# xtcyclist/hash_join_codes_KNL

Measured on AMD Instinct MI355X. Metric: probe Gtuples/s + % HBM roofline, PHJ |R|=64M join |S|=1G, 1/2/4/8 GPU, higher is better.
Workload: dtype u32

## Files before the change

hash_join_codes_knl_amd/csrc/hj_internal.hpp:

```cpp
#pragma once
#include <hip/hip_runtime.h>
#include <stdint.h>
#include <type_traits>
#include "../../include/hjgpu.h"

typedef unsigned long long u64;

constexpr uint32_t HJ_LINE_TUPLES = 16;
constexpr uint32_t HJ_STREAM_UNIT = 256;
constexpr uint32_t HJ_MAX_HEAVY = 128;
struct ScatterConfig { int block, vpt; bool carry; };
struct HjTuning;
ScatterConfig hj_scatter_config(const HjTuning &t, int pass, uint32_t F, bool out_packed);
int hj_scatter_tile(const HjTuning &t, int pass, uint32_t F, bool out_packed);
constexpr int HJ_JOIN_SLICE    = 1 << 16;
constexpr int HJ_JOIN_FILL_GROUPS = 64;
inline size_t hj_join_items_capacity(size_t partitions, size_t outer_rows)
{
    return (partitions + outer_rows / HJ_JOIN_SLICE + 1) * HJ_JOIN_FILL_GROUPS;
}

struct JoinConfig {
    int block, log2slots, batch;
    int slots() const { return 1 << log2slots; }
// ... 8 lines not shown
    bool npj_refhash = false;
    bool no_broadcast = false;
    bool force_chained = false;
    bool scatter_prof = false;
    bool unique = false;
    bool piece_interleave = true;
    bool merged_plan = true;
    int placement = 12;
    int placement_ms = 500;
    bool placement_log = false;
    bool exact_probe_counts = false;
    int probe_slack = 12;
    bool solo = false;
    bool audit = false;
    int hist_min_lds = 0;
    int reserve_cus = 0;
    long long host_batch = -1;
    long long group_from = 300000000, group_inner = 64000000;
    bool group_always = false;
    bool group_device = true;
    int group_slack = 50;
    long long batch_tuples = 0;
    JoinConfig join = {512, 13, 2};
    int scatter_cfg[2][3] = {{0, 0, -1}, {0, 0, -1}};
};
void hj_tuning_from_env(HjTuning *t);
bool hj_tuning_set(HjTuning *t, const char *name, const char *value);
inline const JoinConfig &hj_join_config_of(const HjTuning &t, bool big_tables) { return big_tables ? hj_join_config_big() : t.join; }

struct HjPerDeviceOnce { unsigned char done[64]; };
int hj_allow_dynamic_lds(const void *kernel, int bytes, HjPerDeviceOnce *once);

constexpr uint32_t HJ_MAX_RANGE_ENTRIES = 1u << 24;
constexpr uint32_t HJ_MAX_CHUNKS = 256;
constexpr uint32_t HJ_TICKET_K4 = 0;
constexpr uint32_t HJ_TICKET_K6 = 2 * HJ_MAX_CHUNKS;
constexpr uint32_t HJ_TICKET_MULTI_FILL = 2 * HJ_MAX_CHUNKS + 8;
constexpr uint32_t HJ_TICKET_JOIN = 2 * HJ_MAX_CHUNKS + 10;
constexpr uint32_t HJ_TICKET_JOIN2 = 2 * HJ_MAX_CHUNKS + 12;
constexpr uint32_t HJ_TICKET_JOIN3 = 2 * HJ_MAX_CHUNKS + 14;
constexpr uint32_t HJ_TICKET_WORDS = 2 * HJ_MAX_CHUNKS + 16;
struct Pass1Geom {
    u64 n, part;
#if defined(__HIPCC__)
    __host__ __device__
#endif
    u64 beg(uint32_t c) const { return c >= chunks ? n : part * c; }
    uint32_t chunks;
    uint32_t align;
    uint32_t ranges_per_chunk;
    uint32_t tile;
};
#if defined(__HIPCC__)
__host__ __device__
#endif
inline u64 hj_tiles_of(u64 b, u64 e, uint32_t align, uint32_t tile)
{
    if (e <= b) return 0;
    const u64 gb = (align + b) & ~3ull, ge = align + e;
    return (ge - gb + tile - 1) / tile;
}

struct ScatterArgs {
    const uint32_t *kin, *vin;
// ... 132 lines not shown
int hj_launch_group_result(const hjgpu_result *state, const uint32_t *skew, hjgpu_result *d_result, hipStream_t stream);
int hj_launch_range_base(const uint32_t *range_counts, const u64 *off1, u64 *range_base,
                         uint32_t chunks, uint32_t ranges_per_chunk, uint32_t F1, hipStream_t stream,
                         uint32_t own_first = 0, uint32_t own_count = 0, uint32_t group_bins = 0);
__host__ __device__ inline u64 hj_group_shift(u64 dense_start, uint32_t g)
{
    return ((dense_start + 31) & ~(u64)31) - dense_start + (u64)32 * g;
}
int hj_launch_plan(const PlanArgs &a, hipStream_t stream);
int hj_launch_claimed_pieces(const u64 *off2, const u64 *end2, const u64 *cur2, uint32_t P, u64 *pieces_beg, u64 *pieces_end, hipStream_t stream);
int hj_launch_claimed_desc(const u64 *claim_cursors, u64 cap1, uint32_t F1, uint32_t F2, uint32_t tile2, uint4 *tdesc, uint32_t tdesc_cap,
                           u64 *total, uint32_t *overflow, hipStream_t stream);
struct BatchPlanArgs {
    const uint32_t *range_counts;
    u64 *range_base;
    u64 *boff;
    u64 *tp2b;
    uint4 *tdesc;
    uint32_t tdesc_cap;
    uint32_t ranges, ranges_per_batch, F1, F2, tile2;
};
int hj_launch_batch_plan(const BatchPlanArgs &a, uint32_t batches, hipStream_t stream);
int hj_launch_scatter(const ScatterArgs &a, const HjTuning &t, int cus, hipStream_t stream);
int hj_launch_join(const JoinArgs &a, const HjTuning &t, int cus, hipStream_t stream);
int hj_launch_exscan(const u64 *in, u64 *out, uint32_t n, hipStream_t stream);
int hj_launch_offsets_to_counts(const u64 *off, u64 *counts, uint32_t P, hipStream_t stream);

template <class F>
inline void hj_with_bool(bool b, F &&f)
{
    if (b) f(std::true_type{});
    else f(std::false_type{});
}

int hj_launch_npj_build(const uint32_t *keys, const uint32_t *vals, size_t n, u64 *table,
                        size_t buckets, uint32_t factor, uint32_t *zero_key_flag,
                        int cus, hipStream_t stream, bool line_hash = false);
struct NpjProbeArgs {
    const uint32_t *keys, *vals;
    size_t n;
    const u64 *table;
    size_t buckets;
    uint32_t factor;
    uint32_t line_hash;
    uint32_t unique;
    uint32_t mode;
    hjgpu_result *result;
// ... 104 lines not shown
```

hash_join_codes_knl_amd/csrc/hjgpu_api.hip:

```cpp
#include "hjgpu_ctx.hpp"
#include "hj_device.hpp"

using namespace hjapi;



namespace hjapi {


int fail(hjgpu_ctx *ctx, int status, const char *what, hipError_t e)
{
    if (ctx) {
        if (e != hipSuccess)
            snprintf(ctx->err, sizeof(ctx->err), "%s: %s", what, hipGetErrorString(e));
        else
            snprintf(ctx->err, sizeof(ctx->err), "%s", what);
    }
    return status;
}

static int release(hjgpu_ctx *ctx, void *p)
{
    if (!p) return HJGPU_OK;
    HIPCHK(ctx, hipFree(p));
// ... 160 lines not shown
        m.cur1[r] = take((size_t)C * F1);
        m.tp1[r] = take(C + 1);
        m.seg1[r] = take(C + 1);
        m.tp2[r] = take((size_t)C * F1 + 1);
        m.seg2[r] = take((size_t)F1 + 1);
        m.more[r] = C > 8 ? take(P) : nullptr;
    }
    m.claim_total = take(1);
    m.pieces = take((size_t)4 * P);
    m.slice_prefix = take((size_t)P + 1);
    m.slices = take(P);
    m.item_part = reinterpret_cast<uint32_t *>(take(((size_t)P + items_extra + 2) / 2 + 1));
    for (int r = 0; r < 2; ++r) {
        m.range_counts[r] = reinterpret_cast<uint32_t *>(take((ranges * F1 + 1) / 2));
        m.range_base[r] = take(ranges * F1);
    }
    m.tdesc_cap = tiles2;
    for (int r = 0; r < 2; ++r) m.tdesc[r] = reinterpret_cast<uint4 *>(take(tiles2 * 4));
    m.boff = take(batches * ((size_t)F1 + 1));
    m.tp2b = take(batches * ((size_t)F1 + 1));
    m.tdescb = reinterpret_cast<uint4 *>(take(batches * tdesc_b_cap * 4));
    m.btickets = reinterpret_cast<uint32_t *>(take(batches + 1));
    m.btickets_bytes = (batches + 1) * sizeof(u64);
    m.total_bytes = at * sizeof(u64);
    return m;
}

void choose_fanout(const HjTuning &tune, size_t inner, const hjgpu_phj_params *prm, uint32_t *F1, uint32_t *F2, bool *big_tables)
{
    uint32_t f1 = prm ? prm->fanout1 : 0, f2 = prm ? prm->fanout2 : 0;
    *big_tables = false;
    if (f1 == 0) {
        double target = tune.join.cap() * 0.85;
        double parts = ceil((double)inner / target);
        if (parts > HJGPU_MAX_PARTS) {
            *big_tables = true;
            target = hj_join_config_big().cap() * 0.85;
            parts = ceil((double)inner / target);
        }
        if (parts < 64) parts = 64;
        if (parts > HJGPU_MAX_PARTS) parts = HJGPU_MAX_PARTS;
        if (parts <= 640) { f1 = (uint32_t)parts; f2 = 1; }
        else {
            f1 = 2;
            while ((double)f1 * f1 * 2.0 < parts) f1 <<= 1;
            if (f1 > 256) f1 = 256;
// ... 644 lines not shown
        }
        ja.slice_prefix = m.slice_prefix; ja.slices = m.slices; ja.item_part = m.item_part;
        ja.P = pl.P; ja.chunks = road.pad2 ? 1u : pl.C;
        ja.f1 = pl.f1; ja.F1 = pl.F1; ja.f2 = pl.f2; ja.F2 = pl.F2;
        if (o.pre) { ja.f1 = pl.pre_f1; ja.F1 = pl.pre_F1tot; ja.p1_base = pl.pre_base; }
        ja.tf0 = pl.tf0; ja.tf1 = pl.tf1;
        ja.s_align = 0;
        ja.packed = 1;
        ja.big_tables = pl.big_tables ? 1u : 0u;
        ja.unique = pl.first_match ? 1u : 0u;
        ja.mode = pl.mode;
        ja.result = &st->result;
        ja.work_counter = reinterpret_cast<u64 *>(m.tickets + HJ_TICKET_JOIN);
        ja.work_counter2 = reinterpret_cast<u64 *>(m.tickets + HJ_TICKET_JOIN2);
        ja.work_counter3 = reinterpret_cast<u64 *>(m.tickets + HJ_TICKET_JOIN3);
        ja.multi_fill = m.tickets + HJ_TICKET_MULTI_FILL;
        ja.resume = o.grp ? 1u : 0u;
        join_output(ctx, ja, o.out, bs, bl, st);
        if (marks) {
            ja.build_bits = reinterpret_cast<uint32_t *>(ctx->build_bits.p);
            HIPCHK(ctx, hj_zero_async(ja.build_bits, build_bits_bytes(pl, nn[0]), stream));
            if ((!nn[1] || build_rows) && bs && !o.grp) HIPCHK(ctx, hj_fill_async(ctx->final_offsets.p, 0xFFFFFFFFu, (size_t)workers * sizeof(u64), stream));
        }
        if (nn[1]) CHK(hj_launch_join(ja, ctx->tune, ctx->cus, stream));
        if (build_rows) CHK(hj_launch_build_rows(ja, ctx->tune, ctx->cus, stream));
        else if (marks) CHK(hj_launch_build_unmatched(ja, ctx->tune, ctx->cus, stream));
        if (audit) CHK(hj_audit_copy(reinterpret_cast<const u64 *>(&st->result), audit + 4 * 6, 4, stream));
        return HJGPU_OK;
    }
};

}

int phj_enqueue(hjgpu_ctx *ctx, const PhjPlan &pl, const Rel &R, const Rel &S, hipStream_t stream, const EnqueueOpts &o)
{
    CHK(refuse_capture(ctx, stream));
    if (o.grp && (o.pre || o.stages != PHJ_WHOLE || o.inner_ready)) return fail(ctx, HJGPU_EINVAL, "internal: a device-planned group is a whole join on resident columns");
    if ((o.pre != nullptr) != (pl.pre != 0)) return fail(ctx, HJGPU_EINVAL, "internal: plan and relations disagree about pre-partitioning");
    PhjRun run(ctx, pl, R, S, o, stream);
    const uint32_t workers = (uint32_t)hj_join_workers(ctx->tune, ctx->cus, pl.big_tables);
    u64 bs = 0, bl = 0;
    CHK(setup_output(ctx, o.out, workers, &bs, &bl, pl.mode));

    CHK(run.setup());
    record(ctx, EV_BEGIN, stream);
    CHK(run.begin());
    CHK(run.road.merged ? run.partition_merged() : run.partition_in_turn());
    if (hj_mode_marks_build(pl.mode) && (o.pre || o.stages != PHJ_WHOLE)) return fail(ctx, HJGPU_EINVAL, "internal: a join that marks its build rows is a whole join");
    if (run.road.joins) CHK(run.join(bs, bl, workers));
    record(ctx, EV_JOIN, stream);
    if (bs && run.road.joins && !o.grp) CHK(close_gaps(ctx, o.out, workers, bs, run.st, stream, pl.mode));
    record(ctx, EV_GAPS, stream);
    ctx->stats.fanout1 = pl.F1; ctx->stats.fanout2 = pl.F2; ctx->stats.buckets = 0; ctx->stats.batches = run.batches_used;
    ctx->last_algo = 1;
    return HJGPU_OK;
}

static int finish_from(hjgpu_ctx *ctx, const DevState &h, hjgpu_result *result, const hjgpu_output *out)
{
    if (result) *result = h.result;
    if (h.zero_key) return fail(ctx, HJGPU_EZEROKEY, "NPJ: a build key is 0, the empty-bucket sentinel");
    if (h.overflow) return fail(ctx, HJGPU_EOVERFLOW, "materialised output exceeded its capacity");
    if (out && out->d_keys && h.dense != h.result.count && (h.result.count != 0 || h.dense != 0))
        return fail(ctx, HJGPU_EHIP, "internal: dense length != match count after close_gaps");
    return HJGPU_OK;
}

static int read_state(hjgpu_ctx *ctx, DevState &h, hipStream_t stream)
{
    HIPCHK(ctx, hipMemcpyAsync(&h, ctx->state.p, sizeof(DevState), hipMemcpyDeviceToHost, stream));
    HIPCHK(ctx, hipStreamSynchronize(stream));
    return HJGPU_OK;
}

int finish_blocking(hjgpu_ctx *ctx, hjgpu_result *result, const hjgpu_output *out, hipStream_t stream)
{
    DevState h;
    CHK(read_state(ctx, h, stream));
    return finish_from(ctx, h, result, out);
}

static bool claimed_probe_allowed(const hjgpu_ctx *ctx)
{
// ... 302 lines not shown
    const uint32_t groups = grouped_groups(ctx, inner, outer, nullptr);
    if (groups > 1 && outer) {
        ReserveClock clock(ctx);
        size_t cap_r, cap_s, plan_inner;
        grouped_caps(ctx, groups, inner, outer, &cap_r, &cap_s, &plan_inner);
        CHK(grouped_twins(ctx, group_layout(groups), inner, outer));
        CHK(phj_prepare(ctx, cap_r, cap_s, &prm, 8, &pl, {.plan_inner = plan_inner}));
    } else {
        CHK(phj_prepare(ctx, inner, outer, &prm, 8, &pl));
        if (claimed_probe_allowed(ctx)) CHK(phj_prepare(ctx, inner, outer, &prm, 1, &pl, {.claim_s = true}));
    }
    size_t buckets; uint32_t factor;
    CHK(npj_prepare(ctx, inner, nullptr, &buckets, &factor));
    return HJGPU_OK;
}

static size_t lds_lookup_rows(const HjTuning &tune);
int hjgpu_get_counter(hjgpu_ctx *ctx, const char *name, uint64_t *value)
{
    if (!ctx || !name || !value) return HJGPU_EINVAL;
    if (strcmp(name, "probe_fallbacks") == 0) { *value = ctx->probe_fallbacks; return HJGPU_OK; }
    if (strcmp(name, "probe_exact") == 0) { *value = (ctx->tune.exact_probe_counts || ctx->probe_exact) ? 1u : 0u; return HJGPU_OK; }
    if (strcmp(name, "lookup_lds_rows") == 0) { *value = lds_lookup_rows(ctx->tune); return HJGPU_OK; }
    return fail(ctx, HJGPU_EINVAL, "unknown counter (probe_fallbacks, probe_exact, lookup_lds_rows)");
}

static void fill_reserve(const hjgpu_ctx *ctx, hjgpu_stats *s)
{
    s->ms_reserve = ctx->ms_reserve;
    s->placement_tried = ctx->placement_tried; s->placement_timeboxed = ctx->placement_timeboxed;
    s->placement_fill_ms = ctx->placement_fill_ms; s->placement_search_ms = ctx->placement_search_ms; s->placement_bytes = (uint64_t)ctx->placement_bytes;
}

int hjgpu_get_stats(hjgpu_ctx *ctx, hjgpu_stats *s)
{
    if (!ctx || !s) return HJGPU_EINVAL;
    if (ctx->stats_override) {
        *s = ctx->stats;
        fill_reserve(ctx, s);
        return HJGPU_OK;
    }
    if (ctx->grp_ev_groups) {
        HIPCHK(ctx, hipEventSynchronize(ctx->grp_ev_pass0[2]));
        auto between = [&](hipEvent_t a, hipEvent_t b) -> float { float ms = 0; return hipEventElapsedTime(&ms, a, b) == hipSuccess ? ms : 0.f; };
        hjgpu_stats r = ctx->stats;
        r.ms_histogram = r.ms_plan = r.ms_scatter1 = r.ms_scatter2 = r.ms_join = r.ms_close_gaps = r.ms_build = r.ms_inner_wait = 0;
        for (uint32_t g = 0; g < ctx->grp_ev_groups; ++g) {
// ... 519 lines not shown
                view = *out;
                view.d_keys += acc.dense;
                if (view.d_outer_vals) view.d_outer_vals += acc.dense;
                if (view.d_inner_vals) view.d_inner_vals += acc.dense;
                view.capacity = left / bs * bs; view.block_size = bs;
                vout = &view;
            }
        }
        const Rel g_s = {g_sk + pc[g].s0, g_sv + pc[g].s0, pc[g].sn};
        if (pc[g].rn == 0) {
            CHK(broadcast_enqueue(ctx, {g_rk, g_rv, 0}, g_s, prm, vout, stream, nullptr));
        } else {
            CHK(phj_prepare(ctx, pc[g].rn, pc[g].sn, prm, chunks, &pl));
            CHK(phj_enqueue(ctx, pl, {g_rk + pc[g].r0, g_rv + pc[g].r0, pc[g].rn}, g_s, stream, {.out = vout}));
        }
        DevState h;
        CHK(read_state(ctx, h, stream));
        CHK(hjgpu_get_stats(ctx, &one));
        sum.ms_histogram += one.ms_histogram; sum.ms_plan += one.ms_plan; sum.ms_scatter1 += one.ms_scatter1;
        sum.ms_scatter2 += one.ms_scatter2; sum.ms_join += one.ms_join; sum.ms_close_gaps += one.ms_close_gaps;
        sum.fanout1 = one.fanout1; sum.fanout2 = one.fanout2;
        acc.result.count += h.result.count; acc.result.sum_keys += h.result.sum_keys;
        acc.result.sum_outer_vals += h.result.sum_outer_vals; acc.result.sum_inner_vals += h.result.sum_inner_vals;
        if (h.overflow) { acc.overflow = 1; out_on = false; }
        else if (vout) acc.dense += h.dense;
    }
    HIPCHK(ctx, hipMemcpyAsync(ctx->state.p, &acc, sizeof(DevState), hipMemcpyHostToDevice, stream));
    HIPCHK(ctx, hipStreamSynchronize(stream));
    sum.ms_total = sum.ms_scatter0 + sum.ms_histogram + sum.ms_plan + sum.ms_scatter1 + sum.ms_scatter2 + sum.ms_join + sum.ms_close_gaps;
    sum.groups = G;
    ctx->stats = sum;
    ctx->stats_override = true;
    ctx->last_algo = 1;
    return HJGPU_OK;
}

static void grouped_caps(const hjgpu_ctx *ctx, uint32_t G, size_t inner, size_t outer, size_t *cap_r, size_t *cap_s, size_t *plan_inner)
{
    const size_t slack = (size_t)ctx->tune.group_slack;
    *cap_r = (inner / G + 1) * (100 + slack) / 100 + 65536;
    *cap_s = (outer / G + 1) * (100 + slack) / 100 + 65536;
    *plan_inner = inner / G + inner / G / 10 + 1;
}

static int phj_grouped_device(hjgpu_ctx *ctx, uint32_t G, uint32_t chunks, const Rel &R, const Rel &S, const hjgpu_phj_params *prm,
                              const hjgpu_output *out, hjgpu_result *d_result, hipStream_t stream, hipEvent_t inner_ready)
// ... 212 lines not shown
```

hash_join_codes_knl_amd/csrc/hjgpu_ctx.hpp:

```cpp
#pragma once
#include <hip/hip_runtime.h>
#include <algorithm>
#include <chrono>
#include <functional>
#include <math.h>
#include <stdio.h>
#include <stdlib.h>
#include <string.h>
#include <thread>
#include <vector>

#include "hj_internal.hpp"


struct DevBuf {
    void *p = nullptr;
    size_t cap = 0;
};

namespace hjapi {
struct Rel { const uint32_t *keys = nullptr, *vals = nullptr; size_t rows = 0; };
}

struct DevState {
    hjgpu_result result;
    u64 block_counter;
    u64 dense;
    u64 work_counter;
    uint32_t overflow;
    uint32_t zero_key;
    uint32_t nmoves;
    uint32_t pad;
    u64 work_counter2;
    uint32_t group_skew;
    uint32_t probe_overflow;
};

enum { EV_BEGIN = 0, EV_S_HIST, EV_S_PLAN, EV_S_SC1, EV_S_SC2, EV_WAITED,
       EV_R_HIST, EV_R_PLAN, EV_R_SC1, EV_R_SC2, EV_JOIN, EV_GAPS, EV_COUNT };


struct hjgpu_ctx {
    int device = 0;
    int cus = 0;
    hipDeviceProp_t prop;
    char err[512];
    DevBuf tmp[8];
    DevBuf meta;
    DevBuf table;
    DevBuf state;
    DevBuf moves;
    DevBuf final_offsets;
    DevBuf build_bits;
    hipEvent_t ev[EV_COUNT];
    bool ev_valid[EV_COUNT];
    hjgpu_stats stats;
    int last_algo = -1;
    bool last_lookup = false;
    bool prepared = false;
    size_t prepared_inner = 0, prepared_max_outer = 0;
    unsigned char prepared_plan[128];
    HjTuning tune;
    hipStream_t host_streams[3] = {nullptr, nullptr, nullptr};
    void *host_stage[4] = {nullptr, nullptr, nullptr, nullptr};
    hipEvent_t host_stage_ev[4] = {nullptr, nullptr, nullptr, nullptr};
    hjgpu_output pending_out;
    bool has_pending_out = false;
    bool last_had_output = false;
    uint64_t probe_fallbacks = 0;
    bool probe_exact = false;
    bool rows_plain = false;
    DevBuf grp[4], grp_off;
    bool stats_override = false;
    hipStream_t aux = nullptr;
    hipEvent_t *ev_cur = nullptr;
    std::vector<hipEvent_t> grp_ev;
    uint32_t grp_ev_groups = 0;
    hipEvent_t grp_ev_pass0[3] = {nullptr, nullptr, nullptr};
    struct GroupedCall {
        bool valid = false;
        uint32_t chunks = 1;
        hjapi::Rel R, S;
        bool has_prm = false, has_out = false;
        hjgpu_phj_params prm;
        hjgpu_output out;
        hjgpu_result *d_result = nullptr;
    } grp_last;
    DevBuf audit, audit_lay;
    uint64_t audit_seq = 0;
    struct AuditCheck { int stage; const u64 *tuples, *beg, *end; uint32_t parts; HjAuditHash h; };
    std::vector<AuditCheck> audit_checks;
    float ms_reserve = 0;
// ... 55 lines not shown
uint32_t grouped_groups(const hjgpu_ctx *ctx, size_t inner, size_t outer, const hjgpu_phj_params *prm);
struct GroupLayout { uint32_t G, bins, F0; };
GroupLayout group_layout(uint32_t G);
int grouped_twins(hjgpu_ctx *ctx, const GroupLayout &l, size_t inner, size_t outer);

inline int scatter_cus(const hjgpu_ctx *ctx)
{
    const int n = ctx->cus - ctx->tune.reserve_cus;
    return n < 1 ? 1 : n;
}

inline uint32_t align_of(const void *p) { return (uint32_t)(((uintptr_t)p >> 2) & 3); }

struct MetaLayout {
    u64 *counts[2], *off2[2], *end2[2], *cur2[2], *off1[2], *cur1[2], *tp1[2], *seg1[2], *tp2[2];
    u64 *claim1;
    u64 *claim_total;
    u64 *pieces;
    u64 *seg2[2];
    u64 *more[2];
    u64 *slice_prefix, *slices;
    uint32_t *tickets;
    uint32_t *item_part;
    uint4 *tdesc[2];
    size_t tdesc_cap;
    uint32_t *range_counts[2];
    u64 *range_base[2];
    u64 *boff, *tp2b;
    uint4 *tdescb;
    uint32_t *btickets;
    size_t btickets_bytes;
    size_t counts_bytes;
    size_t total_bytes;
};
MetaLayout carve(void *base, uint32_t C, uint32_t F1, uint32_t P, size_t ranges, size_t items_extra = 0,
                 size_t tiles2 = 0, size_t batches = 0, size_t tdesc_b_cap = 0);
ScatterArgs scatter_pass1(const hjgpu_ctx *ctx, const MetaLayout &m, int r, const Pass1Geom &geom, uint32_t F, uint32_t factor,
                          const uint32_t *kin, const uint32_t *vin, uint32_t *kout, uint32_t *vout);
PlanArgs plan_args(const hjgpu_ctx *ctx, const MetaLayout &m, uint32_t C, uint32_t F1, uint32_t F2, uint32_t tile1, uint32_t tile2, bool unique,
                   uint32_t mask);
void join_output(const hjgpu_ctx *ctx, JoinArgs &ja, const hjgpu_output *out, u64 bs, u64 bl, DevState *st);
int close_gaps(hjgpu_ctx *ctx, const hjgpu_output *out, uint32_t workers, u64 bs, DevState *st, hipStream_t stream, uint32_t mode = HJ_MODE_INNER);
int check_join_mode(hjgpu_ctx *ctx, uint32_t flags);
int refuse_join_mode(hjgpu_ctx *ctx, uint32_t flags, const char *entry);
void choose_fanout(const HjTuning &tune, size_t inner, const hjgpu_phj_params *prm, uint32_t *F1, uint32_t *F2, bool *big_tables);
void record(hjgpu_ctx *ctx, int which, hipStream_t s);
// ... 84 lines not shown
```

hash_join_codes_knl_amd/csrc/join_kernels.hip:

```cpp
#include "hj_device.hpp"
#include "hj_internal.hpp"
#include "hj_emit.hpp"
#include "hj_lookup_sel.hpp"

constexpr int hj_join_wgs_per_cu(int block, int log2slots)
{
    const int by_lds = (160 * 1024) / ((1 << log2slots) * 8 + 1024 + 9 * 1024), by_threads = 2048 / block;
    const int n = by_lds < by_threads ? by_lds : by_threads;
    return n < 1 ? 1 : n;
}
constexpr int hj_join_waves_per_simd(int block, int log2slots)
{
    const int w = hj_join_wgs_per_cu(block, log2slots) * (block / 64) / 4;
    return w < 1 ? 1 : w;
}

template <int LOG2SLOTS>
__device__ __forceinline__ uint2 hj_cuckoo_slots(uint32_t key, uint32_t tf0, uint32_t tf1)
{
    const uint32_t a1 = (key * tf0) >> (32 - LOG2SLOTS);
    return make_uint2(a1, (a1 + (((key * tf1) >> (32 - LOG2SLOTS)) | 1u)) & ((1u << LOG2SLOTS) - 1));
}

#ifndef HJ_EMIT4
#define HJ_EMIT4 1
#endif
struct hj_tail_pass {
    __device__ uint32_t operator()(const uint32_t (&)[4], const uint32_t (&)[4], const bool (&)[4]) const { return 0u; }
};
struct hj_mark_pass {
    __device__ uint32_t operator()(const uint32_t (&)[4], const uint32_t (&)[4], const bool (&)[4]) const { return 0u; }
};

template <bool ON, uint32_t WORDS>
struct SlotBits {
    static __device__ __forceinline__ uint32_t *get() { __shared__ uint32_t bits[WORDS]; return bits; }
};
template <uint32_t WORDS>
struct SlotBits<false, WORDS> {
    static __device__ __forceinline__ uint32_t *get() { return nullptr; }
};

template <int BLOCK, int LOG2SLOTS, int BATCH, bool PACKED, bool UNIQUE, bool DEDUP, bool NTROWS, int MODE>
__device__ __forceinline__ void join_body(JoinArgs a)
{
    constexpr bool LEFTISH = MODE == HJ_MODE_LEFT_OUTER || MODE == HJ_MODE_FULL_OUTER;
    constexpr bool MARKING = MODE == HJ_MODE_MARK;
    constexpr bool KEEPB = MODE == HJ_MODE_RIGHT_OUTER || MODE == HJ_MODE_FULL_OUTER || MARKING;
    static_assert(UNIQUE || !DEDUP || MODE == HJ_MODE_LEFT_OUTER || MARKING, "DEDUP is the multi-fill half of a _UNIQUE or left / full outer join");
    static_assert(MODE == HJ_MODE_INNER || ((UNIQUE || LEFTISH || KEEPB) && NTROWS),
                  "semi- and anti-joins walk to the first match; rows non-temporal");
    static_assert(!(KEEPB && UNIQUE), "right and full outer joins walk to every copy of a build key");
    static_assert(!(KEEPB && DEDUP) || MARKING, "the multi-fill items of a full outer join are marked by a launch of its own");
    constexpr bool SPLIT = UNIQUE || LEFTISH || MARKING;
    if (DEDUP && a.multi_fill && *a.multi_fill == 0) return;
    constexpr uint32_t SLOTS = 1u << LOG2SLOTS;
    constexpr uint32_t MASK = SLOTS - 1;
    constexpr uint32_t CAP = SLOTS / 2;
    constexpr int SHIFT = 32 - LOG2SLOTS;
    constexpr int NW = BLOCK / 64;
    constexpr int RB = 8;
    constexpr int CUCKOO_MAX_EVICTIONS = 64;
    __shared__ u64 tab64[SLOTS];
    __shared__ u64 red[4][NW];
    __shared__ u64 wave_cursor[NW];
    __shared__ uint32_t cuckoo_failed;
    constexpr uint32_t MATCHED_WORDS = (DEDUP && !MARKING) ? (HJ_JOIN_SLICE + 64) / 32 + 2 : 1;
    __shared__ uint32_t matched[MATCHED_WORDS];
    constexpr bool dedup = DEDUP;
    uint2 *tab = reinterpret_cast<uint2 *>(tab64);
    uint32_t *const slot_bits = SlotBits<KEEPB, SLOTS / 32>::get();

    const int tid = threadIdx.x;
    const int wave = tid >> 6;
    const uint32_t P = a.P, C = a.chunks;
    const u64 total_items = a.slice_prefix[P];
    const uint4 *__restrict__ sk4 = reinterpret_cast<const uint4 *>(PACKED ? a.sk : a.sk - a.s_align);
    const uint4 *__restrict__ sv4 = reinterpret_cast<const uint4 *>(PACKED ? a.sk : a.sv - a.s_align);
// ... 405 lines not shown
                        for (uint32_t n = 0; n < SLOTS; ++n) {
                            const uint32_t tk = tab[slot].x;
                            if (tk == k) { hit = (slot_bits[slot >> 5] >> (slot & 31)) & 1u; break; }
                            if (tk == empty) break;
                            slot = (slot + step) & MASK;
                        }
                    }
                }
                const u64 m = __ballot(hit);
                const uint32_t lane = hj_lane(), sh = (uint32_t)at & 31u;
                if (m && (sh == 0 || lane == 0)) {
                    const uint32_t w = (uint32_t)((m >> lane) << sh);
                    if (w) atomicOr(&a.build_bits[at >> 5], w);
                }
            }
            seen += len;
        }
    };

    __shared__ u64 d_item[2], d_rb[2], d_rn[2];
    __shared__ u64 d_rows_beg[2], d_rows_end[2];
    __shared__ uint32_t d_q[2], d_slice[2], d_nslices[2];
    auto claim = [&](int slot) {
        const u64 w = atomicAdd(a.work_counter, 1ull);
        d_item[slot] = w;
        if (w < total_items) {
            const uint32_t nq = a.item_part[w];
            d_q[slot] = nq;
            const u64 shape = a.slices[nq];
            const uint32_t nslices = (uint32_t)shape, groups = (uint32_t)(shape >> 32);
            const uint32_t t = (uint32_t)(w - a.slice_prefix[nq]);
            const u64 rb = a.roff[nq], rn = a.rend[nq] - rb;
            d_rb[slot] = rb;
            d_rn[slot] = rn;
            d_nslices[slot] = nslices | (a.s_pieces << 24);
            u64 rows = rn;
            for (uint32_t c = 1; c < C; ++c) rows += a.rend[(u64)c * P + nq] - a.roff[(u64)c * P + nq];
            if (groups == 1) {
                d_slice[slot] = t;
                d_rows_beg[slot] = 0;
                d_rows_end[slot] = rows;
            } else {
                const uint32_t group = t / nslices;
                d_slice[slot] = t - group * nslices;
                const uint32_t fills = (uint32_t)((rows + CAP - 1) >> (LOG2SLOTS - 1));
                const uint32_t per_group = (fills + groups - 1) / groups;
                d_rows_beg[slot] = min(rows, (u64)group * per_group * CAP);
// ... 104 lines not shown
            }
        }
        if constexpr (LEFTISH) {
            if (DEDUP || rows_beg >= rows_end) {
                probe_item(slice, nslices, hj_tail_pass{});
                if (DEDUP) __syncthreads();
            }
        }
        if (rows_beg >= rows_end) __syncthreads();
        par ^= 1;
    }

    if (a.ok) hj_leave_cursor(a.final_offsets, wave_cursor);

    hj_add_to_result(red, a.result, acc_n, acc_k, acc_o, acc_i);
}

template <int BLOCK, int LOG2SLOTS, int BATCH, bool PACKED, bool UNIQUE, bool DEDUP = false, bool NTROWS = true>
__global__ __launch_bounds__(BLOCK, hj_join_waves_per_simd(BLOCK, LOG2SLOTS)) void join_kernel(JoinArgs a)
{
    join_body<BLOCK, LOG2SLOTS, BATCH, PACKED, UNIQUE, DEDUP, NTROWS, HJ_MODE_INNER>(a);
}

template <int BLOCK, int LOG2SLOTS, int BATCH, bool PACKED, int MODE, bool DEDUP>
__global__ __launch_bounds__(BLOCK, hj_join_waves_per_simd(BLOCK, LOG2SLOTS)) void exists_probe_kernel(JoinArgs a)
{
    join_body<BLOCK, LOG2SLOTS, BATCH, PACKED, true, DEDUP, true, MODE>(a);
}

template <int BLOCK, int LOG2SLOTS, int BATCH, bool PACKED, bool UNIQUE, bool DEDUP>
__global__ __launch_bounds__(BLOCK, hj_join_waves_per_simd(BLOCK, LOG2SLOTS)) void outer_probe_kernel(JoinArgs a)
{
    join_body<BLOCK, LOG2SLOTS, BATCH, PACKED, UNIQUE, DEDUP, true, HJ_MODE_LEFT_OUTER>(a);
}

template <int BLOCK, int LOG2SLOTS, int BATCH, bool PACKED>
__global__ __launch_bounds__(BLOCK, hj_join_waves_per_simd(BLOCK, LOG2SLOTS)) void right_probe_kernel(JoinArgs a)
{
    join_body<BLOCK, LOG2SLOTS, BATCH, PACKED, false, false, true, HJ_MODE_RIGHT_OUTER>(a);
}

template <int BLOCK, int LOG2SLOTS, int BATCH, bool PACKED>
__global__ __launch_bounds__(BLOCK, hj_join_waves_per_simd(BLOCK, LOG2SLOTS)) void full_probe_kernel(JoinArgs a)
{
    join_body<BLOCK, LOG2SLOTS, BATCH, PACKED, false, false, true, HJ_MODE_FULL_OUTER>(a);
}
// ... 258 lines not shown
    u64 split = (u64)grid * 4 / pieces;
    split = split < 1 ? 1 : split > 4096 ? 4096 : split;
    if (c.block == 512) hipLaunchKernelGGL((build_unmatched_kernel<512>), dim3(grid), dim3(512), 0, stream, a, (uint32_t)split);
    else if (c.block == 1024) hipLaunchKernelGGL((build_unmatched_kernel<1024>), dim3(grid), dim3(1024), 0, stream, a, (uint32_t)split);
    else return HJGPU_EINVAL;
    return hipGetLastError() == hipSuccess ? HJGPU_OK : HJGPU_EHIP;
}

int hj_launch_build_rows(const JoinArgs &a, const HjTuning &t, int cus, hipStream_t stream)
{
    if (!hj_mode_reports_build(a.mode) || !a.packed || !a.build_bits || a.P < 1 || a.chunks == 0 || (a.ok && (!a.final_offsets || !a.oiv))) return HJGPU_EINVAL;
    const JoinConfig &c = hj_join_config_of(t, a.big_tables != 0);
    const int grid = join_grid(cus, c);
    const u64 pieces = (u64)a.P * a.chunks;
    u64 split = (u64)grid * 4 / pieces;
    split = split < 1 ? 1 : split > 4096 ? 4096 : split;
    const uint32_t flip = a.mode == HJ_MODE_RIGHT_SEMI ? ~0u : 0u;
    if (c.block == 512) hipLaunchKernelGGL((build_rows_kernel<512>), dim3(grid), dim3(512), 0, stream, a, (uint32_t)split, flip);
    else if (c.block == 1024) hipLaunchKernelGGL((build_rows_kernel<1024>), dim3(grid), dim3(1024), 0, stream, a, (uint32_t)split, flip);
    else return HJGPU_EINVAL;
    return hipGetLastError() == hipSuccess ? HJGPU_OK : HJGPU_EHIP;
}

int hj_launch_join(const JoinArgs &a, const HjTuning &t, int cus, hipStream_t stream)
{
    if ((a.P < 2 && !a.broadcast) || a.P < 1 || a.chunks == 0) return HJGPU_EINVAL;
    const JoinConfig &c = hj_join_config_of(t, a.big_tables != 0);
    JoinArgs b = a;
    b.force_chained = t.force_chained ? 1u : 0u;
    b.unique = (a.unique || t.unique) ? 1u : 0u;
    if ((b.unique || b.mode) && !b.work_counter2) return HJGPU_EINVAL;
    if (hj_mode_keeps_build(b.mode) && (b.unique || !b.build_bits)) return HJGPU_EINVAL;
    if (hj_mode_reports_build(b.mode) && !b.build_bits) return HJGPU_EINVAL;
    const int grid = join_grid(cus, c);
    if (c.block == 512 && c.log2slots == 13) return launch_join_at<512, 13, true>(b, c.batch, grid, stream);
    if (c.block == 1024 && c.log2slots == 14) return launch_join_at<1024, 14, true>(b, c.batch, grid, stream);
    if (c.block == 256 && c.log2slots == 12) return launch_join_at<256, 12, false>(b, c.batch, grid, stream);
    return HJGPU_EINVAL;
}

template <int CTRL>
__device__ __forceinline__ uint32_t lds_dpp(uint32_t x)
{
    return (uint32_t)__builtin_amdgcn_mov_dpp((int)x, CTRL, 0xF, 0xF, true);
}

template <bool VALS, bool BITS>
__device__ __forceinline__ void lds_lookup_leave(const LdsLookupArgs &a, u64 v, const uint32_t (&kc)[4], const uint32_t (&res)[4], uint32_t nib,
                                                 u64 &acc_n, u64 &acc_k, u64 &acc_i)
{
    const u64 n = a.n, g = v << 2;
#pragma unroll
    for (int j = 0; j < 4; ++j) {
        const bool hit = (nib >> j) & 1u;
        acc_n += hit ? 1u : 0u; acc_k += hit ? kc[j] : 0u; acc_i += hit ? res[j] : 0u;
    }
    if constexpr (VALS) {
// ... 345 lines not shown
```

hash_join_codes_knl_amd/csrc/partition_kernels.hip:

```cpp
#include "hj_device.hpp"
#include "hj_internal.hpp"
#include <stdlib.h>
#include <stdio.h>
#include <string.h>
#include <type_traits>

#ifndef HJ_K6_STORE
#define HJ_K6_STORE 1
#endif
__device__ __forceinline__ void k6_store16(u64 *p, uint4 v)
{
#if HJ_K6_STORE == 1 || HJ_K6_STORE == 3
    typedef uint32_t v4u_t __attribute__((ext_vector_type(4)));
    v4u_t t = {v.x, v.y, v.z, v.w};
    __builtin_nontemporal_store(t, reinterpret_cast<v4u_t *>(p));
#elif HJ_K6_STORE == 2
    __hip_atomic_store(p, (u64)v.x | ((u64)v.y << 32), __ATOMIC_RELAXED, __HIP_MEMORY_SCOPE_SYSTEM);
    __hip_atomic_store(p + 1, (u64)v.z | ((u64)v.w << 32), __ATOMIC_RELAXED, __HIP_MEMORY_SCOPE_SYSTEM);
#else
    *reinterpret_cast<uint4 *>(p) = v;
#endif
}
template <bool NT>
__device__ __forceinline__ void k6_store8(u64 *p, u64 v)
// ... 1444 lines not shown
        return true;
    }
    if (is("batch_tuples")) {
        char *end = nullptr;
        const long long x = strtoll(value, &end, 10);
        if (end == value || *end) return false;
        t->batch_tuples = x;
        return true;
    }
    if (is("range_tiles")) {
        char *end = nullptr;
        const long x = strtol(value, &end, 10);
        if (end == value || *end || x < 0 || x > (1 << 20)) return false;
        t->range_tiles = (int)x;
        return true;
    }
    if (is("join_cfg")) {
        int b, l, u;
        if (!*value) { t->join = JoinConfig{512, 13, 2}; return true; }
        if (sscanf(value, "%d,%d,%d", &b, &l, &u) != 3) return false;
        t->join = JoinConfig{b, l, u};
        return true;
    }
    if (is("scatter_cfg") || is("scatter2_cfg")) {
        int *o = t->scatter_cfg[is("scatter_cfg") ? 0 : 1];
        int b, v, c = -1;
        if (!*value) { o[0] = 0; o[1] = 0; o[2] = -1; return true; }
        if (sscanf(value, "%d,%d,%d", &b, &v, &c) < 2 || b <= 0 || v <= 0) return false;
        o[0] = b; o[1] = v; o[2] = c;
        return true;
    }
    return false;
}

void hj_tuning_from_env(HjTuning *t)
{
    static const char *const names[] = {"dense2", "npj_refhash", "no_broadcast", "force_chained", "scatter_prof",
                                        "unique", "merged_plan", "piece_interleave", "range_tiles", "batch_tuples", "group_from", "group_inner", "group_always", "group_device", "group_slack", "host_batch", "placement", "placement_ms", "placement_log", "audit", "solo", "exact_probe_counts", "probe_slack", "hist_min_lds", "reserve_cus", "join_cfg", "scatter_cfg", "scatter2_cfg"};
    for (const char *n : names) {
        char env[64] = "HJGPU_";
        size_t at = strlen(env);
        for (const char *c = n; *c && at + 1 < sizeof(env); ++c) env[at++] = (char)((*c >= 'a' && *c <= 'z') ? *c - 32 : *c);
        env[at] = 0;
        const char *v = getenv(env);
        if (v && *v && !hj_tuning_set(t, n, v))
            fprintf(stderr, "hjgpu: ignoring malformed %s=%s\n", env, v);
    }
}
```

Before: 122.3.

## Add specialized aggregate-only join kernel with deferred fallback for hard partitions

Adds an inner-join kernel for aggregate-only output. Each block builds a cuckoo table of a single-slice partition in LDS, prefetches the next partition's build tuples, and accumulates count and sums with 32-bit split adders instead of 64-bit adds. Partitions that are multi-slice, too large, or fail cuckoo insertion are put on a device list and handled by a second launch of the general join kernel, which claims only those items. This drops the generic join's materialisation and mode machinery on the common path, at the cost of an extra kernel launch, a second LDS table build for deferred items, and more template instances.

```diff
diff --git a/hash_join_codes_knl_amd/csrc/hj_internal.hpp b/hash_join_codes_knl_amd/csrc/hj_internal.hpp
--- a/hash_join_codes_knl_amd/csrc/hj_internal.hpp
+++ b/hash_join_codes_knl_amd/csrc/hj_internal.hpp
@@ -54,6 +54,8 @@
     int group_slack = 50;
     long long batch_tuples = 0;
     JoinConfig join = {512, 13, 2};
+    bool agg_join = true;
+    int agg_block = 1024, agg_batch = 1;
     int scatter_cfg[2][3] = {{0, 0, -1}, {0, 0, -1}};
 };
 void hj_tuning_from_env(HjTuning *t);
@@ -71,7 +73,8 @@
 constexpr uint32_t HJ_TICKET_JOIN = 2 * HJ_MAX_CHUNKS + 10;
 constexpr uint32_t HJ_TICKET_JOIN2 = 2 * HJ_MAX_CHUNKS + 12;
 constexpr uint32_t HJ_TICKET_JOIN3 = 2 * HJ_MAX_CHUNKS + 14;
-constexpr uint32_t HJ_TICKET_WORDS = 2 * HJ_MAX_CHUNKS + 16;
+constexpr uint32_t HJ_TICKET_AGG_DEFERRED = 2 * HJ_MAX_CHUNKS + 16;
+constexpr uint32_t HJ_TICKET_WORDS = 2 * HJ_MAX_CHUNKS + 18;
 struct Pass1Geom {
     u64 n, part;
 #if defined(__HIPCC__)
@@ -250,7 +253,9 @@
 };
 int hj_launch_batch_plan(const BatchPlanArgs &a, uint32_t batches, hipStream_t stream);
 int hj_launch_scatter(const ScatterArgs &a, const HjTuning &t, int cus, hipStream_t stream);
-int hj_launch_join(const JoinArgs &a, const HjTuning &t, int cus, hipStream_t stream);
+struct AggDeferred { uint32_t *count, *items, *total; };
+bool hj_agg_join_built(int block, int batch);
+int hj_launch_join(const JoinArgs &a, const HjTuning &t, int cus, hipStream_t stream, const AggDeferred *agg = nullptr);
 int hj_launch_exscan(const u64 *in, u64 *out, uint32_t n, hipStream_t stream);
 int hj_launch_offsets_to_counts(const u64 *off, u64 *counts, uint32_t P, hipStream_t stream);
 
diff --git a/hash_join_codes_knl_amd/csrc/hjgpu_api.hip b/hash_join_codes_knl_amd/csrc/hjgpu_api.hip
--- a/hash_join_codes_knl_amd/csrc/hjgpu_api.hip
+++ b/hash_join_codes_knl_amd/csrc/hjgpu_api.hip
@@ -206,6 +206,7 @@
     m.tdescb = reinterpret_cast<uint4 *>(take(batches * tdesc_b_cap * 4));
     m.btickets = reinterpret_cast<uint32_t *>(take(batches + 1));
     m.btickets_bytes = (batches + 1) * sizeof(u64);
+    m.agg_items = reinterpret_cast<uint32_t *>(take(((size_t)P + items_extra + 2) / 2 + 1));
     m.total_bytes = at * sizeof(u64);
     return m;
 }
@@ -896,7 +897,8 @@
             HIPCHK(ctx, hj_zero_async(ja.build_bits, build_bits_bytes(pl, nn[0]), stream));
             if ((!nn[1] || build_rows) && bs && !o.grp) HIPCHK(ctx, hj_fill_async(ctx->final_offsets.p, 0xFFFFFFFFu, (size_t)workers * sizeof(u64), stream));
         }
-        if (nn[1]) CHK(hj_launch_join(ja, ctx->tune, ctx->cus, stream));
+        const AggDeferred agg = {m.tickets + HJ_TICKET_AGG_DEFERRED, m.agg_items, &st->agg_deferred};
+        if (nn[1]) CHK(hj_launch_join(ja, ctx->tune, ctx->cus, stream, &agg));
         if (build_rows) CHK(hj_launch_build_rows(ja, ctx->tune, ctx->cus, stream));
         else if (marks) CHK(hj_launch_build_unmatched(ja, ctx->tune, ctx->cus, stream));
         if (audit) CHK(hj_audit_copy(reinterpret_cast<const u64 *>(&st->result), audit + 4 * 6, 4, stream));
@@ -933,6 +935,7 @@
 static int finish_from(hjgpu_ctx *ctx, const DevState &h, hjgpu_result *result, const hjgpu_output *out)
 {
     if (result) *result = h.result;
+    ctx->agg_join_deferred = h.agg_deferred;
     if (h.zero_key) return fail(ctx, HJGPU_EZEROKEY, "NPJ: a build key is 0, the empty-bucket sentinel");
     if (h.overflow) return fail(ctx, HJGPU_EOVERFLOW, "materialised output exceeded its capacity");
     if (out && out->d_keys && h.dense != h.result.count && (h.result.count != 0 || h.dense != 0))
@@ -1281,7 +1284,8 @@
     if (strcmp(name, "probe_fallbacks") == 0) { *value = ctx->probe_fallbacks; return HJGPU_OK; }
     if (strcmp(name, "probe_exact") == 0) { *value = (ctx->tune.exact_probe_counts || ctx->probe_exact) ? 1u : 0u; return HJGPU_OK; }
     if (strcmp(name, "lookup_lds_rows") == 0) { *value = lds_lookup_rows(ctx->tune); return HJGPU_OK; }
-    return fail(ctx, HJGPU_EINVAL, "unknown counter (probe_fallbacks, probe_exact, lookup_lds_rows)");
+    if (strcmp(name, "agg_join_deferred") == 0) { *value = ctx->agg_join_deferred; return HJGPU_OK; }
+    return fail(ctx, HJGPU_EINVAL, "unknown counter (probe_fallbacks, probe_exact, lookup_lds_rows, agg_join_deferred)");
 }
 
 static void fill_reserve(const hjgpu_ctx *ctx, hjgpu_stats *s)
@@ -1847,6 +1851,7 @@
         sum.fanout1 = one.fanout1; sum.fanout2 = one.fanout2;
         acc.result.count += h.result.count; acc.result.sum_keys += h.result.sum_keys;
         acc.result.sum_outer_vals += h.result.sum_outer_vals; acc.result.sum_inner_vals += h.result.sum_inner_vals;
+        acc.agg_deferred += h.agg_deferred;
         if (h.overflow) { acc.overflow = 1; out_on = false; }
         else if (vout) acc.dense += h.dense;
     }
diff --git a/hash_join_codes_knl_amd/csrc/hjgpu_ctx.hpp b/hash_join_codes_knl_amd/csrc/hjgpu_ctx.hpp
--- a/hash_join_codes_knl_amd/csrc/hjgpu_ctx.hpp
+++ b/hash_join_codes_knl_amd/csrc/hjgpu_ctx.hpp
@@ -34,6 +34,8 @@
     u64 work_counter2;
     uint32_t group_skew;
     uint32_t probe_overflow;
+    uint32_t agg_deferred;
+    uint32_t pad1;
 };
 
 enum { EV_BEGIN = 0, EV_S_HIST, EV_S_PLAN, EV_S_SC1, EV_S_SC2, EV_WAITED,
@@ -68,6 +70,7 @@
     bool has_pending_out = false;
     bool last_had_output = false;
     uint64_t probe_fallbacks = 0;
+    uint64_t agg_join_deferred = 0;
     bool probe_exact = false;
     bool rows_plain = false;
     DevBuf grp[4], grp_off;
@@ -169,6 +172,7 @@
     u64 *slice_prefix, *slices;
     uint32_t *tickets;
     uint32_t *item_part;
+    uint32_t *agg_items;
     uint4 *tdesc[2];
     size_t tdesc_cap;
     uint32_t *range_counts[2];
diff --git a/hash_join_codes_knl_amd/csrc/join_kernels.hip b/hash_join_codes_knl_amd/csrc/join_kernels.hip
--- a/hash_join_codes_knl_amd/csrc/join_kernels.hip
+++ b/hash_join_codes_knl_amd/csrc/join_kernels.hip
@@ -41,8 +41,8 @@
     static __device__ __forceinline__ uint32_t *get() { return nullptr; }
 };
 
-template <int BLOCK, int LOG2SLOTS, int BATCH, bool PACKED, bool UNIQUE, bool DEDUP, bool NTROWS, int MODE>
-__device__ __forceinline__ void join_body(JoinArgs a)
+template <int BLOCK, int LOG2SLOTS, int BATCH, bool PACKED, bool UNIQUE, bool DEDUP, bool NTROWS, int MODE, bool DEFERRED = false>
+__device__ __forceinline__ void join_body(JoinArgs a, const uint32_t *def_count = nullptr, const uint32_t *def_items = nullptr)
 {
     constexpr bool LEFTISH = MODE == HJ_MODE_LEFT_OUTER || MODE == HJ_MODE_FULL_OUTER;
     constexpr bool MARKING = MODE == HJ_MODE_MARK;
@@ -54,6 +54,7 @@
     static_assert(!(KEEPB && DEDUP) || MARKING, "the multi-fill items of a full outer join are marked by a launch of its own");
     constexpr bool SPLIT = UNIQUE || LEFTISH || MARKING;
     if (DEDUP && a.multi_fill && *a.multi_fill == 0) return;
+    if constexpr (DEFERRED) { if (*def_count == 0) return; }
     constexpr uint32_t SLOTS = 1u << LOG2SLOTS;
     constexpr uint32_t MASK = SLOTS - 1;
     constexpr uint32_t CAP = SLOTS / 2;
@@ -505,7 +506,8 @@
     __shared__ u64 d_rows_beg[2], d_rows_end[2];
     __shared__ uint32_t d_q[2], d_slice[2], d_nslices[2];
     auto claim = [&](int slot) {
-        const u64 w = atomicAdd(a.work_counter, 1ull);
+        u64 w = atomicAdd(a.work_counter, 1ull);
+        if constexpr (DEFERRED) w = w < *def_count ? (u64)def_items[w] : total_items;
         d_item[slot] = w;
         if (w < total_items) {
             const uint32_t nq = a.item_part[w];
@@ -656,6 +658,13 @@
     join_body<BLOCK, LOG2SLOTS, BATCH, PACKED, UNIQUE, DEDUP, NTROWS, HJ_MODE_INNER>(a);
 }
 
+template <int BLOCK, int LOG2SLOTS, int BATCH, bool PACKED>
+__global__ __launch_bounds__(BLOCK, hj_join_waves_per_simd(BLOCK, LOG2SLOTS)) void deferred_join_kernel(JoinArgs a, const uint32_t *def_count,
+                                                                                                      const uint32_t *def_items)
+{
+    join_body<BLOCK, LOG2SLOTS, BATCH, PACKED, false, false, true, HJ_MODE_INNER, true>(a, def_count, def_items);
+}
+
 template <int BLOCK, int LOG2SLOTS, int BATCH, bool PACKED, int MODE, bool DEDUP>
 __global__ __launch_bounds__(BLOCK, hj_join_waves_per_simd(BLOCK, LOG2SLOTS)) void exists_probe_kernel(JoinArgs a)
 {
@@ -960,7 +969,241 @@
     return hipGetLastError() == hipSuccess ? HJGPU_OK : HJGPU_EHIP;
 }
 
-int hj_launch_join(const JoinArgs &a, const HjTuning &t, int cus, hipStream_t stream)
+struct AggJoinArgs { JoinArgs j; AggDeferred d; };
+
+__device__ __forceinline__ void agg_add(uint32_t &lo, uint32_t &hi, uint32_t x)
+{
+    hi += __builtin_add_overflow(lo, x, &lo) ? 1u : 0u;
+}
+
+template <int BLOCK, int LOG2SLOTS, int BATCH>
+__global__ __launch_bounds__(BLOCK, hj_join_waves_per_simd(BLOCK, LOG2SLOTS)) void agg_join_kernel(AggJoinArgs aa)
+{
+    const JoinArgs &a = aa.j;
+    constexpr uint32_t SLOTS = 1u << LOG2SLOTS;
+    constexpr uint32_t CAP = SLOTS / 2;
+    constexpr int SHIFT = 32 - LOG2SLOTS;
+    constexpr int NW = BLOCK / 64;
+    constexpr int RB = (CAP + BLOCK - 1) / BLOCK;
+    constexpr int CUCKOO_MAX_EVICTIONS = 64;
+    constexpr uint32_t DEFER = 0xFFFFFFFFu;
+    constexpr bool PREFETCH = BLOCK == 512;
+    __shared__ u64 tab64[SLOTS];
+    __shared__ u64 red[4][NW];
+    __shared__ uint32_t cuckoo_failed;
+    __shared__ u64 d_item[2], d_rb[2];
+    __shared__ uint32_t d_q[2], d_slice[2], d_nslices[2], d_rn[2];
+
+    const uint32_t tid = threadIdx.x;
+    const uint32_t P = a.P;
+    const u64 total_items = a.slice_prefix[P];
+    const uint4 *__restrict__ sk4 = reinterpret_cast<const uint4 *>(a.sk);
+    const u64 *__restrict__ r64 = reinterpret_cast<const u64 *>(a.rk);
+    u64 acc_n = 0;
+    uint32_t k_lo = 0, k_hi = 0, o_lo = 0, o_hi = 0, i_lo = 0, i_hi = 0;
+
+    auto claim = [&](int slot) {
+        const u64 w = atomicAdd(a.work_counter, 1ull);
+        d_item[slot] = w;
+        if (w < total_items) {
+            const uint32_t nq = a.item_part[w];
+            const u64 shape = a.slices[nq];
+            const u64 rb = a.roff[nq], rn = a.rend[nq] - rb;
+            d_q[slot] = nq;
+            d_rb[slot] = rb;
+            d_slice[slot] = (uint32_t)(w - a.slice_prefix[nq]);
+            d_nslices[slot] = (uint32_t)shape | (a.s_pieces << 24);
+            d_rn[slot] = ((uint32_t)(shape >> 32) != 1 || rn > CAP) ? DEFER : (uint32_t)rn;
+        }
+    };
+    auto defer = [&](u64 w) {
+        const uint32_t at = atomicAdd(aa.d.count, 1u);
+        hj_store(aa.d.items + at, (uint32_t)w);
+        atomicAdd(aa.d.total, 1u);
+    };
+
+    u64 br[RB];
+    bool have = false;
+#pragma unroll
+    for (int j = 0; j < RB; ++j) br[j] = 0;
+    int par = 0;
+    if (tid == 0) claim(0);
+    __syncthreads();
+    for (;;) {
+        const u64 w = hj_uniform(d_item[par]);
+        if (w >= total_items) break;
+        const uint32_t q = hj_uniform(d_q[par]);
+        const uint32_t slice = hj_uniform(d_slice[par]), nslices_word = hj_uniform(d_nslices[par]);
+        const uint32_t rn = hj_uniform(d_rn[par]);
+        const u64 rb = hj_uniform(d_rb[par]);
+        if (tid == 0) claim(par ^ 1);
+        if (rn == DEFER || rn == 0) {
+            if (tid == 0 && rn == DEFER) defer(w);
+            have = false;
+            __syncthreads();
+            par ^= 1;
+            continue;
+        }
+        if (!PREFETCH || !have) {
+#pragma unroll
+            for (int j = 0; j < RB; ++j) {
+                const uint32_t i = (uint32_t)j * BLOCK + tid;
+                br[j] = 0;
+                if (i < rn) br[j] = r64[rb + i];
+            }
+        }
+        have = false;
+        uint32_t empty = 0;
+        while ((hj_hash(empty, a.f1, a.F1) - a.p1_base) * a.F2 + hj_hash(empty, a.f2, a.F2) == q) ++empty;
+        uint32_t other = empty + 1;
+        while ((hj_hash(other, a.f1, a.F1) - a.p1_base) * a.F2 + hj_hash(other, a.f2, a.F2) == q) ++other;
+        const u64 EMPTY64 = (u64)empty;
+        uint32_t tf0 = a.tf0, tf1 = a.tf1;
+        for (int attempt = 0; attempt < 2; ++attempt) {
+            for (uint32_t i = tid; i < SLOTS; i += BLOCK) tab64[i] = EMPTY64;
+            if (tid == 0) cuckoo_failed = 0;
+            __syncthreads();
+#pragma unroll
+            for (int j = 0; j < RB; ++j) {
+                if ((uint32_t)j * BLOCK + tid >= rn) continue;
+                u64 cur = br[j];
+                uint32_t loc = ((uint32_t)cur * tf0) >> SHIFT;
+                int it = 0;
+                for (; it < CUCKOO_MAX_EVICTIONS; ++it) {
+                    const u64 old = atomicExch(&tab64[loc], cur);
+                    if ((uint32_t)old == empty) break;
+                    const uint2 a12 = hj_cuckoo_slots<LOG2SLOTS>((uint32_t)old, tf0, tf1);
+                    loc = (loc == a12.x) ? a12.y : a12.x;
+                    cur = old;
+                }
+                if (it == CUCKOO_MAX_EVICTIONS) cuckoo_failed = 1;
+            }
+            __syncthreads();
+            if (attempt == 1 || !hj_uniform(cuckoo_failed)) break;
+            __syncthreads();
+            const uint32_t t = tf0; tf0 = tf1; tf1 = t;
+        }
+        if constexpr (PREFETCH) {
+            const uint32_t nrn = hj_uniform(d_rn[par ^ 1]);
+            if (hj_uniform(d_item[par ^ 1]) < total_items && nrn != DEFER && nrn != 0) {
+                const u64 nrb = hj_uniform(d_rb[par ^ 1]);
+                have = true;
+#pragma unroll
+                for (int j = 0; j < RB; ++j) {
+                    const uint32_t i = (uint32_t)j * BLOCK + tid;
+                    br[j] = 0;
+                    if (i < nrn) br[j] = r64[nrb + i];
+                }
+            }
+        }
+        if (hj_uniform(cuckoo_failed)) {
+            if (tid == 0) defer(w);
+        } else {
+            const uint32_t nslices = nslices_word & 0xFFFFFFu, pieces = 1 + (nslices_word >> 24);
+            for (uint32_t c = 0; c < pieces; ++c) {
+                const u64 b = a.soff[(u64)c * P + q], e = a.send[(u64)c * P + q];
+                const u64 len = e - b;
+                if (len == 0) continue;
+                const u64 gb = a.s_align + b + (len * slice) / nslices;
+                const u64 ge = a.s_align + b + (len * (slice + 1)) / nslices;
+                const u64 base = gb & ~3ull;
+                const uint32_t lead = (uint32_t)(gb - base), end = (uint32_t)(ge - base);
+                const uint4 *__restrict__ s4 = sk4 + (base >> 1);
+                for (uint32_t o0 = tid * 4; o0 < end; o0 += (uint32_t)BLOCK * 4 * BATCH) {
+                    uint4 kk[BATCH], vv[BATCH];
+#pragma unroll
+                    for (int u = 0; u < BATCH; ++u) {
+                        const uint32_t o = o0 + (uint32_t)u * BLOCK * 4;
+                        kk[u] = make_uint4(0, 0, 0, 0); vv[u] = kk[u];
+                        if (o < end) { kk[u] = hj_load_nt(s4 + (o >> 1)); vv[u] = hj_load_nt(s4 + (o >> 1) + 1); }
+                    }
+#pragma unroll
+                    for (int u = 0; u < BATCH; ++u) {
+                        const uint32_t o = o0 + (uint32_t)u * BLOCK * 4;
+                        if (o >= end) break;
+                        uint32_t key[4] = {kk[u].x, kk[u].z, vv[u].x, vv[u].z};
+                        const uint32_t val[4] = {kk[u].y, kk[u].w, vv[u].y, vv[u].w};
+                        if (o < lead || o + 4 > end) {
+#pragma unroll
+                            for (int j = 0; j < 4; ++j) if (o + j < lead || o + j >= end) key[j] = other;
+                        }
+                        u64 t1[4], t2[4];
+#pragma unroll
+                        for (int j = 0; j < 4; ++j) {
+                            const uint2 at = hj_cuckoo_slots<LOG2SLOTS>(key[j], tf0, tf1);
+                            t1[j] = tab64[at.x];
+                            t2[j] = tab64[at.y];
+                        }
+                        uint32_t n = 0;
+                        bool twice = false;
+#pragma unroll
+                        for (int j = 0; j < 4; ++j) {
+                            const bool h1 = (uint32_t)t1[j] == key[j], h2 = (uint32_t)t2[j] == key[j];
+                            const bool hit = h1 || h2;
+                            n += hit ? 1u : 0u;
+                            agg_add(k_lo, k_hi, hit ? key[j] : 0u);
+                            agg_add(o_lo, o_hi, hit ? val[j] : 0u);
+                            agg_add(i_lo, i_hi, hit ? (uint32_t)((h1 ? t1[j] : t2[j]) >> 32) : 0u);
+                            twice = twice || (h1 && h2);
+                        }
+                        if (twice) {
+#pragma unroll
+                            for (int j = 0; j < 4; ++j) {
+                                if ((uint32_t)t1[j] == key[j] && (uint32_t)t2[j] == key[j]) {
+                                    n += 1u;
+                                    agg_add(k_lo, k_hi, key[j]); agg_add(o_lo, o_hi, val[j]); agg_add(i_lo, i_hi, (uint32_t)(t2[j] >> 32));
+                                }
+                            }
+                        }
+                        acc_n += n;
+                    }
+                }
+            }
+        }
+        __syncthreads();
+        par ^= 1;
+    }
+    hj_add_to_result(red, a.result, (u64)acc_n, ((u64)k_hi << 32) | k_lo, ((u64)o_hi << 32) | o_lo, ((u64)i_hi << 32) | i_lo);
+}
+
+static const struct { int block, batch; } AGG_JOIN_BUILT[] = {{512, 1}, {512, 2}, {768, 1}, {768, 2}, {1024, 1}};
+
+bool hj_agg_join_built(int block, int batch)
+{
+    for (const auto &g : AGG_JOIN_BUILT) if (g.block == block && g.batch == batch) return true;
+    return false;
+}
+
+static bool hj_agg_join_applies(const JoinArgs &b, const HjTuning &t, const JoinConfig &c, const AggDeferred *agg)
+{
+    return t.agg_join && agg && agg->count && agg->items && agg->total && b.mode == HJ_MODE_INNER && !b.unique && b.packed && !b.ok &&
+           b.chunks == 1 && !b.broadcast && !b.force_chained && !b.big_tables && c.block == 512 && c.log2slots == 13 && c.batch == 2 &&
+           hj_agg_join_built(t.agg_block, t.agg_batch);
+}
+
+template <int B, int U>
+static void launch_agg_join_at(const AggJoinArgs &aa, int grid, hipStream_t stream)
+{
+    hipLaunchKernelGGL((agg_join_kernel<B, 13, U>), dim3(grid), dim3(B), 0, stream, aa);
+}
+
+static int launch_agg_join(const JoinArgs &b, const HjTuning &t, const AggDeferred &agg, int grid, hipStream_t stream)
+{
+    const AggJoinArgs aa = {b, agg};
+    const int block = t.agg_block, batch = t.agg_batch;
+    if (block == 512 && batch == 1) launch_agg_join_at<512, 1>(aa, grid, stream);
+    else if (block == 512 && batch == 2) launch_agg_join_at<512, 2>(aa, grid, stream);
+    else if (block == 768 && batch == 1) launch_agg_join_at<768, 1>(aa, grid, stream);
+    else if (block == 768 && batch == 2) launch_agg_join_at<768, 2>(aa, grid, stream);
+    else if (block == 1024 && batch == 1) launch_agg_join_at<1024, 1>(aa, grid, stream);
+    else return HJGPU_EINVAL;
+    JoinArgs d = b;
+    d.work_counter = b.work_counter2;
+    hipLaunchKernelGGL((deferred_join_kernel<512, 13, 2, true>), dim3(grid), dim3(512), 0, stream, d, (const uint32_t *)agg.count, (const uint32_t *)agg.items);
+    return hipGetLastError() == hipSuccess ? HJGPU_OK : HJGPU_EHIP;
+}
+
+int hj_launch_join(const JoinArgs &a, const HjTuning &t, int cus, hipStream_t stream, const AggDeferred *agg)
 {
     if ((a.P < 2 && !a.broadcast) || a.P < 1 || a.chunks == 0) return HJGPU_EINVAL;
     const JoinConfig &c = hj_join_config_of(t, a.big_tables != 0);
@@ -971,6 +1214,7 @@
     if (hj_mode_keeps_build(b.mode) && (b.unique || !b.build_bits)) return HJGPU_EINVAL;
     if (hj_mode_reports_build(b.mode) && !b.build_bits) return HJGPU_EINVAL;
     const int grid = join_grid(cus, c);
+    if (hj_agg_join_applies(b, t, c, agg)) return b.work_counter2 ? launch_agg_join(b, t, *agg, grid, stream) : HJGPU_EINVAL;
     if (c.block == 512 && c.log2slots == 13) return launch_join_at<512, 13, true>(b, c.batch, grid, stream);
     if (c.block == 1024 && c.log2slots == 14) return launch_join_at<1024, 14, true>(b, c.batch, grid, stream);
     if (c.block == 256 && c.log2slots == 12) return launch_join_at<256, 12, false>(b, c.batch, grid, stream);
diff --git a/hash_join_codes_knl_amd/csrc/partition_kernels.hip b/hash_join_codes_knl_amd/csrc/partition_kernels.hip
--- a/hash_join_codes_knl_amd/csrc/partition_kernels.hip
+++ b/hash_join_codes_knl_amd/csrc/partition_kernels.hip
@@ -1490,6 +1490,14 @@
         t->join = JoinConfig{b, l, u};
         return true;
     }
+    if (is("agg_join")) return parse_flag(value, &t->agg_join);
+    if (is("agg_join_cfg")) {
+        int b, u;
+        if (!*value) { t->agg_block = HjTuning().agg_block; t->agg_batch = HjTuning().agg_batch; return true; }
+        if (sscanf(value, "%d,%d", &b, &u) != 2 || !hj_agg_join_built(b, u)) return false;
+        t->agg_block = b; t->agg_batch = u;
+        return true;
+    }
     if (is("scatter_cfg") || is("scatter2_cfg")) {
         int *o = t->scatter_cfg[is("scatter_cfg") ? 0 : 1];
         int b, v, c = -1;
@@ -1504,7 +1512,7 @@
 void hj_tuning_from_env(HjTuning *t)
 {
     static const char *const names[] = {"dense2", "npj_refhash", "no_broadcast", "force_chained", "scatter_prof",
-                                        "unique", "merged_plan", "piece_interleave", "range_tiles", "batch_tuples", "group_from", "group_inner", "group_always", "group_device", "group_slack", "host_batch", "placement", "placement_ms", "placement_log", "audit", "solo", "exact_probe_counts", "probe_slack", "hist_min_lds", "reserve_cus", "join_cfg", "scatter_cfg", "scatter2_cfg"};
+                                        "unique", "merged_plan", "piece_interleave", "range_tiles", "batch_tuples", "group_from", "group_inner", "group_always", "group_device", "group_slack", "host_batch", "placement", "placement_ms", "placement_log", "audit", "solo", "exact_probe_counts", "probe_slack", "hist_min_lds", "reserve_cus", "join_cfg", "agg_join", "agg_join_cfg", "scatter_cfg", "scatter2_cfg"};
     for (const char *n : names) {
         char env[64] = "HJGPU_";
         size_t at = strlen(env);
```

New measurement: 121.2. Within noise of the previous version (-0.9%).
